# EricPedley/ORB_SLAM3_ROS2

Measured on AMD Instinct MI355X. Metric: frames/sec ORB extract+match @640×480; KF/sec LocalBA (50 KF, 2k pts), higher is better.
Workload: dtype u8; 1 GPU; C2: 640x480, 8-level pyramid, 1000 feat/frame, FAST 20/7, batch=1 per camera stream; ORBextractor::operator() + brute-force Hamming match to the camera's previous frame; step=one frame on each of 16 independent camera streams, parallelism=replicas x1 (no collective); 16 camera streams per GPU, batch 1 each, cameras=16

## Files before the change

orb_slam3_ros2_amd/csrc/extract.cpp:

```cpp
#include "extract.h"

#include <algorithm>
#include <cstdlib>
#include <cstring>
#include <map>
#include <memory>
#include <mutex>
#include <vector>

#include "devbuf.h"
#include "graph_cache.h"
#include "orbhip_kernels.h"
#include "stage.h"

#define HIPOK(x) ORBHIP_HIPOK(" extract", x)

namespace orbhip {
namespace {

struct Plan {
    HostPlan hp;
    DevBuf<ExtractPlan> d_plan;
    DevBuf<CellGeom> d_cells;
    DevBuf<int> d_xofs, d_xalpha, d_yofs, d_ybeta, d_disc, d_cone_tab, d_cone_hi_tab, d_bands, d_flow_dep;
// ... 9 lines not shown
};
std::mutex g_plan_m;
std::map<PlanKey, std::weak_ptr<Plan>>& plan_cache() {
    static auto* m = new std::map<PlanKey, std::weak_ptr<Plan>>();
    return *m;
}

int cone_hi_threads() {
    static const int t = std::getenv("ORBHIP_CONE_HI_THREADS") ? std::atoi(std::getenv("ORBHIP_CONE_HI_THREADS")) : 256;
    return (t == 512 || t == 1024) ? t : 256;
}

template <typename T>
hipError_t upload(DevBuf<T>& d, const std::vector<T>& v) {
    if (v.empty()) return hipSuccess;
    const hipError_t e = d.ensure(v.size());
    return e != hipSuccess ? e : hipMemcpy(d.p, v.data(), v.size() * sizeof(T), hipMemcpyHostToDevice);
}

int upload_plan(Plan& pl) {
    const HostPlan& hp = pl.hp;
    HIPOK(pl.d_plan.ensure(1));
    HIPOK(hipMemcpy(pl.d_plan.p, &hp.h, sizeof(ExtractPlan), hipMemcpyHostToDevice));
    HIPOK(upload(pl.d_cells, hp.cells));
    HIPOK(upload(pl.d_xofs, hp.xofs));
    HIPOK(upload(pl.d_xalpha, hp.xalpha));
    HIPOK(upload(pl.d_yofs, hp.yofs));
    HIPOK(upload(pl.d_ybeta, hp.ybeta));
    HIPOK(upload(pl.d_disc, hp.disc));
    HIPOK(upload(pl.d_otab, hp.otab));
    HIPOK(upload(pl.d_bands, hp.bands));
    HIPOK(upload(pl.d_flow_dep, hp.flow_dep));
    HIPOK(upload(pl.d_cone_hi, hp.cone_hi));
    HIPOK(upload(pl.d_cone_hi_tab, hp.cone_hi_tab));
    HIPOK(upload(pl.d_cone, hp.cone));
    HIPOK(upload(pl.d_cone_tab, hp.cone_tab));
    return ORBHIP_OK;
}

struct RunSwitches {
    int oct_fast, oct_max_dh;
    bool no_cone;
    bool cone_hi;
    bool pack;
    bool flow;
};
RunSwitches read_run_switches() {
    auto is1 = [](const char* name) {
        const char* e = std::getenv(name);
        return e && e[0] == '1';
    };
    const char* e_dh = std::getenv("ORBHIP_OCTREE_DH");
    RunSwitches s;
    s.oct_fast = is1("ORBHIP_OCTREE_SWEEP") ? 0 : 1;
    s.oct_max_dh = e_dh ? std::max(1, std::min(6, std::atoi(e_dh))) : 6;
    s.no_cone = std::getenv("ORBHIP_NO_CONE") != nullptr;
    s.cone_hi = is1("ORBHIP_CONE_HI");
    s.pack = is1("ORBHIP_CAND_PACK");
    s.flow = is1("ORBHIP_RZ_FLOW");
    return s;
}

}

struct ExtractWorkspace {
    int device = 0;
    const orbhip_orb_params* prm = nullptr;
    const OrbTables* tab = nullptr;
    StageTimer* timer = nullptr;
// ... 61 lines not shown
    HIPOK(ws->grow(ws->d_pyr, (size_t)B * P.pyr_bytes));
    HIPOK(ws->grow(ws->d_cand, (size_t)B * P.n_slots_total));
    HIPOK(ws->grow(ws->d_cprim, (size_t)B * P.n_cells_total * kCandPrim));
    HIPOK(ws->grow(ws->d_kscratch, (size_t)B * P.n_slots_total));
    HIPOK(ws->grow(ws->d_nscratch, (size_t)B * P.n_slots_total));
    HIPOK(ws->grow(ws->d_cand_cnt, (size_t)B * P.n_cells_total));
    HIPOK(ws->grow(ws->d_cand_off, (size_t)B * P.n_cells_total));
    HIPOK(ws->grow(ws->d_cand_fill, (size_t)B * kMaxLevels));
    if (pl->hp.flow_nbt) {
        const uint64_t was = ws->gen;
        HIPOK(ws->grow(ws->d_flow, kFlowCtl + (size_t)B * pl->hp.flow_nbt));
        if (ws->gen != was) HIPOK(hipMemset(ws->d_flow.p, 0, ws->d_flow.n * sizeof(int)));
    }
    HIPOK(ws->grow(ws->d_lvl_kp, (size_t)B * P.kp_slots_total));
    HIPOK(ws->grow(ws->d_lvl_cnt, (size_t)B * P.n_levels));
    HIPOK(ws->grow(ws->d_lvl_nlap, (size_t)B * P.n_levels));
    HIPOK(ws->grow(ws->d_err, 4));
    return ORBHIP_OK;
}

static void launch_pyramid(ExtractWorkspace* ws, Plan* pl, FrameBufs& fb, int B, const RunSwitches& sw, bool flow_on,
                           hipStream_t st) {
    const ExtractPlan& P = pl->hp.h;
    StageTimer& tm = *ws->timer;
    static const size_t cone_max = std::getenv("ORBHIP_CONE_MAX_WG")
                                       ? (size_t)std::atol(std::getenv("ORBHIP_CONE_MAX_WG"))
                                       : (size_t)1024;
    const bool cone_path = pl->hp.cone_tiles && !sw.no_cone && (size_t)B * pl->hp.cone_tiles <= cone_max;
    const bool cone_hi = !cone_path && pl->hp.cone_hi_tiles && sw.cone_hi;
    fb.stamp = (cone_path && tm.stage == 1 && tm.dstamp && tm.n < StageTimer::kCap) ? tm.dstamp + tm.n : nullptr;
    if (cone_path) {
        static const int cone_nt = [] {
            const char* e = std::getenv("ORBHIP_CONE_NT");
            const int v = e ? std::atoi(e) : 1024;
            return (v == 256 || v == 512) ? v : 1024;
        }();
        launch_pyr_cone(pl->d_plan.p, pl->hp.cone_tiles, pl->hp.cone_lds, fb, B, pl->d_cone.p, pl->d_cone_tab.p,
                        pl->hp.cone_tab_stride, st, 0, cone_nt, pl->d_xofs.p, pl->d_xalpha.p, pl->d_yofs.p,
                        pl->d_ybeta.p);
    } else if (flow_on) {
        PyrFlow fa{};
        fa.ctl = ws->d_flow.p;
        fa.flags = ws->d_flow.p + kFlowCtl;
        fa.dep = (const int2*)pl->d_flow_dep.p;
        for (int l = 0; l <= kMaxLevels; l++) fa.boff[l] = pl->hp.flow_boff[l];
        fa.B = B;
        fa.nbt = pl->hp.flow_nbt;
        fa.pyr_limit = (int)((int64_t)B * P.pyr_bytes);
        launch_pyr_flow(pl->d_plan.p, fb, pl->d_xofs.p, pl->d_xalpha.p, pl->d_yofs.p, pl->d_ybeta.p, fa, st);
    } else {
        const bool bands = !cone_hi && pl->hp.nbands > 0;
        const int lr = cone_hi ? kConeHiStart + 1 : (bands ? kBandStart + 1 : P.n_levels);
        for (int l = 1; l < lr; l++)
            launch_resize(pl->d_plan.p, P, fb, B, l, pl->d_xofs.p, pl->d_xalpha.p, pl->d_yofs.p, pl->d_ybeta.p,
                          st);
        if (cone_hi)
            launch_pyr_cone(pl->d_plan.p, pl->hp.cone_hi_tiles, pl->hp.cone_hi_lds, fb, B, pl->d_cone_hi.p,
                            pl->d_cone_hi_tab.p, pl->hp.cone_hi_tab_stride, st, kConeHiStart, cone_hi_threads(),
                            pl->d_xofs.p, pl->d_xalpha.p, pl->d_yofs.p, pl->d_ybeta.p);
        if (bands)
            launch_resize_bands(pl->d_plan.p, pl->hp.nbands, fb, B, kBandStart, (const int2*)pl->d_bands.p,
                                pl->d_xofs.p, pl->d_xalpha.p, pl->d_yofs.p, pl->d_ybeta.p, st);
    }
}

static int run_extract(ExtractWorkspace* ws, Plan* pl, const uint8_t* d_imgs, int B, int stride, int64_t fstride,
                       int lap0, int lap1, orbhip_kp* d_kps, uint8_t* d_desc, int cap, int32_t* d_n, int32_t* d_mono,
                       hipStream_t st) {
    const ExtractPlan& P = pl->hp.h;
    (void)hipGetLastError();
    int rc = ensure_batch(ws, pl, B);
    if (rc) return rc;
    const RunSwitches sw = read_run_switches();
    const bool flow_on = sw.flow && pl->hp.flow_nbt > 0 && (int64_t)B * P.pyr_bytes < (1ll << 31);
    GraphKey key;
    key.add(1).add((uint64_t)sw.oct_fast).add((uint64_t)sw.oct_max_dh).add((uint64_t)sw.no_cone)
        .add((uint64_t)sw.cone_hi).add((uint64_t)flow_on).add((uint64_t)sw.pack).add((uint64_t)ws->fast_nt).ptr(pl)
        .ptr(d_imgs).add((uint64_t)B).add((uint64_t)stride).add((uint64_t)fstride).add((uint64_t)lap0)
        .add((uint64_t)lap1).ptr(d_kps).ptr(d_desc).add((uint64_t)cap).ptr(d_n).ptr(d_mono).ptr(st)
        .ptr(ws).add(ws->gen);
    return ws->graphs->run(key, st, ws->timer->stage != 0, [&](hipStream_t st) -> int {
        FrameBufs fb;
        fb.in = d_imgs; fb.in_stride = stride; fb.in_fstride = fstride; fb.pyr = ws->d_pyr.p;
        StageTimer& tm = *ws->timer;
        const StageScope scope(tm);
        tm.begin(1, st);
        launch_pyramid(ws, pl, fb, B, sw, flow_on, st);
        tm.end(1, st);
        tm.begin(2, st);
        CandPack cp;
        cp.prim = ws->d_cprim.p;
// ... 192 lines not shown
```

orb_slam3_ros2_amd/csrc/extract_kernels.hip:

```cpp
#include <hip/hip_runtime.h>
#include <cstdlib>
#include <type_traits>

#include "../../include/orbhip.h"
#include "dev_attr.h"
#include "../../include/orbhip_pattern.h"
#include "orbhip_device.h"
#include "orbhip_kernels.h"
#include "orbhip_plan.h"

namespace orbhip {

__constant__ __attribute__((visibility("hidden"))) signed char kPattern[256 * 4] = ORBHIP_BIT_PATTERN_31_INIT;

ORBHIP_TRACE_UNIT(extract)

struct ImgRef {
    const uint8_t* p;
    int pitch;
};

__device__ __forceinline__ ImgRef level_img(const ExtractPlan* __restrict__ P, const FrameBufs& fb, int f, int l) {
    if (l == 0) return ImgRef{fb.in + (int64_t)f * fb.in_fstride, fb.in_stride};
    return ImgRef{fb.pyr + (int64_t)f * P->pyr_bytes + P->lv[l].pyr_off, P->lv[l].pitch};
// ... 279 lines not shown
                        typedef unsigned int u32x4v __attribute__((ext_vector_type(4)));
                        const u32x4v u = {v.x, v.y, v.z, v.w};
                        __builtin_amdgcn_raw_buffer_store_b128(u, prs, obase + (dyb + r) * pitch + c, 0, 16);
                    }
                    wave_lds_only();
                }
            }
            asm volatile("s_waitcnt vmcnt(0)" ::: "memory");
            __syncthreads();
            if (tid == 0)
                __hip_atomic_store((ex_gint*)(fl + a.boff[l] + b), gen + 1, __ATOMIC_RELAXED,
                                   __HIP_MEMORY_SCOPE_AGENT);
            if (tr_k < 32) { TR_PHASE(7, 2 * tr_k + 1) }
            tr_k++;
        }
    }
    TR_END(7)
    if (tid == 0 && atomicAdd(ctl + kFlowQ, 1) == (int)gridDim.x - 1) {
        for (int i = 0; i <= kFlowQ; i++)
            __hip_atomic_store((ex_gint*)(ctl + i), 0, __ATOMIC_RELAXED, __HIP_MEMORY_SCOPE_AGENT);
        __hip_atomic_store((ex_gint*)(ctl + kFlowQ + 1), gen + 1, __ATOMIC_RELAXED, __HIP_MEMORY_SCOPE_AGENT);
    }
}

__device__ __forceinline__ int small_div(int i, float inv_d) { return (int)(((float)i + 0.5f) * inv_d); }

__device__ __forceinline__ void wait_vm_all() { asm volatile("s_waitcnt vmcnt(0)" ::: "memory"); }
__device__ __forceinline__ void lds_only_barrier() {
    asm volatile("s_waitcnt lgkmcnt(0)" ::: "memory");
    __builtin_amdgcn_s_barrier();
    asm volatile("" ::: "memory");
}

__device__ __forceinline__ void pyr_cone_body(const ExtractPlan* __restrict__ P, const FrameBufs& fb,
                                              const ConeRect* __restrict__ rects, const int* __restrict__ ctab,
                                              int tab_stride, uint8_t* __restrict__ cone, int tile, int f, int s0) {
    TR_BEGIN()
    const int L = P->n_levels, tid = threadIdx.x, nt = blockDim.x;
    const ConeRect* R = rects + (size_t)tile * kMaxLevels;
    static_assert(sizeof(ConeRect) == 16 && kMaxLevels * 4 <= 64 && (kMaxLevels & (kMaxLevels - 1)) == 0, "4 dwords per level");
    const uint32_t rdw = ((const uint32_t*)R)[threadIdx.x & (4 * kMaxLevels - 1)];
    auto rect = [&](int l) -> ConeRect {
        const uint32_t d0 = (uint32_t)__builtin_amdgcn_readlane((int)rdw, 4 * l),
                       d1 = (uint32_t)__builtin_amdgcn_readlane((int)rdw, 4 * l + 1),
                       d2 = (uint32_t)__builtin_amdgcn_readlane((int)rdw, 4 * l + 2),
                       d3 = (uint32_t)__builtin_amdgcn_readlane((int)rdw, 4 * l + 3);
        return ConeRect{(int16_t)(d0 & 0xFFFF), (int16_t)(d0 >> 16), (int16_t)(d1 & 0xFFFF), (int16_t)(d1 >> 16),
                        (int16_t)(d2 & 0xFFFF), (int16_t)(d2 >> 16), (int16_t)(d3 & 0xFFFF), (int16_t)(d3 >> 16)};
    };
    int boff[kMaxLevels], toff[kMaxLevels];
    int tot = 0;
    const ConeRect Rs0 = rect(s0);
    const int P0 = (Rs0.nx1 - Rs0.nx0 + 6) & ~3;
    for (int l = s0; l < L; l++) {
        const ConeRect r = rect(l);
        boff[l] = tot;
        tot += ((l == s0 ? P0 : (r.nx1 - r.nx0)) * (r.ny1 - r.ny0) + 15) & ~15;
    }
    int sh0 = 0;
    int* tab = (int*)(cone + tot);
    int ttot = 0;
    for (int l = s0 + 1; l < L; l++) {
        toff[l] = ttot;
        const ConeRect r = rect(l);
        ttot += 2 * (r.nx1 - r.nx0) + 3 * (r.ny1 - r.ny0);
    }
    const int* gt = ctab + (size_t)tile * tab_stride;
    auto tab_at = [&](int i) -> int { return gt[i]; };
    TR_PHASE(0, 20)
    {
        const ImgRef in0 = level_img(P, fb, f, s0);
        const ConeRect r = Rs0;
        const int nw = r.nx1 - r.nx0, nh = r.ny1 - r.ny0;
        const uint8_t* src0 = in0.p + (int64_t)r.ny0 * in0.pitch + r.nx0;
        const bool dw = ((in0.pitch & 3) == 0) && ((((uintptr_t)in0.p) & 3) == 0);
        if (dw) sh0 = (int)(((uintptr_t)src0) & 3);
        const int nwd = dw ? (nw + sh0 + 3) >> 2 : 0;
        const int tot0 = dw ? nwd * nh : nw * nh;
        const float inv_n = 1.0f / (float)(dw ? nwd : nw);
        uint8_t* lv0 = cone + boff[s0];
        if (dw && tot0 <= 1024 && ttot <= 2 * 1024 && nt == 1024) {
            const uint32_t* s4 = (const uint32_t*)(src0 - sh0);
            const int p4 = in0.pitch >> 2;
            int tv[2];
#pragma unroll
            for (int u = 0; u < 2; u++) tv[u] = gt[min(tid + 1024 * u, ttot - 1)];
            const int i = min(tid, tot0 - 1);
            const int y = small_div(i, inv_n), x = i - y * nwd;
            const uint32_t v = s4[(int64_t)y * p4 + x];
#pragma unroll
            for (int u = 0; u < 2; u++)
                if (tid + 1024 * u < ttot) tab[tid + 1024 * u] = tv[u];
            if (tid < tot0) ((uint32_t*)lv0)[y * (P0 >> 2) + x] = v;
            TR_PHASE(0, 21)
        } else if (dw) {
            const uint32_t* s4 = (const uint32_t*)(src0 - sh0);
            const int p4 = in0.pitch >> 2;
            constexpr int U = 8;
            for (int i0 = tid; i0 < ttot; i0 += U * nt) {
                int v[U];
#pragma unroll
                for (int u = 0; u < U; u++) v[u] = tab_at(min(i0 + u * nt, ttot - 1));
#pragma unroll
                for (int u = 0; u < U; u++)
                    if (i0 + u * nt < ttot) tab[i0 + u * nt] = v[u];
            }
            for (int i0 = tid; i0 < tot0; i0 += U * nt) {
                uint32_t v[U];
                int o[U];
#pragma unroll
                for (int u = 0; u < U; u++) {
                    const int i = min(i0 + u * nt, tot0 - 1);
                    const int y = small_div(i, inv_n), x = i - y * nwd;
                    v[u] = s4[(int64_t)y * p4 + x];
                    o[u] = y * (P0 >> 2) + x;
                }
#pragma unroll
                for (int u = 0; u < U; u++)
                    if (i0 + u * nt < tot0) ((uint32_t*)lv0)[o[u]] = v[u];
            }
        } else {
            for (int i = tid; i < ttot; i += nt) tab[i] = tab_at(i);
            for (int i = tid; i < tot0; i += nt) {
                const int y = small_div(i, inv_n), x = i - y * nw;
                lv0[y * P0 + x] = src0[(int64_t)y * in0.pitch + x];
            }
        }
    }
    __syncthreads();
    TR_PHASE(0, 0)
    for (int l = s0 + 1; l < L; l++) {
        const LevelGeom& D = P->lv[l];
        const ConeRect r = rect(l), rp = rect(l - 1);
        const int nw = r.nx1 - r.nx0, nh = r.ny1 - r.ny0, nwp = l == s0 + 1 ? P0 : rp.nx1 - rp.nx0;
        const int* t = tab + toff[l];
        const uint8_t* src = cone + boff[l - 1] + (l == s0 + 1 ? sh0 : 0);
        uint8_t* dst = fb.pyr + (int64_t)f * P->pyr_bytes + D.pyr_off;
        const float inv_nw = 1.0f / (float)nw;
        const bool noclamp = D.rz_noclamp != 0;
        for (int i = tid; i < nw * nh; i += nt) {
            const int yy = small_div(i, inv_nw), xx = i - yy * nw;
            const int x = r.nx0 + xx, y = r.ny0 + yy;
            const int sx = t[xx] - rp.nx0;
            const uint8_t* S0 = src + (t[2 * nw + 3 * yy] - rp.ny0) * nwp;
            const uint8_t* S1 = src + (t[2 * nw + 3 * yy + 1] - rp.ny0) * nwp;
            int h0, h1;
            if (x < D.xmax) {
                const int aa = t[nw + xx];
                const int a0 = (int)(short)(aa & 0xFFFF), a1 = (int)(short)(aa >> 16);
                h0 = S0[sx] * a0 + S0[sx + 1] * a1;
                h1 = S1[sx] * a0 + S1[sx + 1] * a1;
            } else {
                h0 = S0[sx] * 2048;
                h1 = S1[sx] * 2048;
            }
            const int bb = t[2 * nw + 3 * yy + 2];
            const int b0 = (int)(short)(bb & 0xFFFF), b1 = (int)(short)(bb >> 16);
            int v;
            if (x < D.vend && noclamp) {
                v = ((__mul24(h0 >> 4, b0) >> 16) + (__mul24(h1 >> 4, b1) >> 16) + 2) >> 2;
            } else if (x < D.vend) {
                int s0 = min(max(h0 >> 4, -32768), 32767);
                int s1 = min(max(h1 >> 4, -32768), 32767);
                int tt = ((s0 * b0) >> 16) + ((s1 * b1) >> 16);
                tt = min(max(tt, -32768), 32767);
                v = (tt + 2) >> 2;
            } else {
                v = (h0 * b0 + h1 * b1 + (1 << 21)) >> 22;
            }
            const uint8_t u = (uint8_t)(v < 0 ? 0 : (v > 255 ? 255 : v));
            cone[boff[l] + i] = u;
            if (x >= r.ox0 && x < r.ox1 && y >= r.oy0 && y < r.oy1) dst[(int64_t)y * D.pitch + x] = u;
        }
        lds_only_barrier();
        TR_PHASE(0, l)
    }
    TR_END(0)
}

__global__ __launch_bounds__(1024) void k_pyr_cone(const ExtractPlan* __restrict__ P, FrameBufs fb,
                                                   const ConeRect* __restrict__ rects, const int* __restrict__ ctab,
                                                   int tab_stride, int xrun, int s0) {
    extern __shared__ __attribute__((aligned(16))) uint8_t cone[];
    if (fb.stamp && threadIdx.x == 0) atomicMin(fb.stamp, (unsigned long long)__builtin_amdgcn_s_memrealtime());
    const int X = gridDim.x, lg = xcd_runs(blockIdx.x + X * blockIdx.y, X * gridDim.y, xrun < 0 ? X : xrun);
    pyr_cone_body(P, fb, rects, ctab, tab_stride, cone, lg % X, lg / X, s0);
    if (fb.stamp) {
        __syncthreads();
        if (threadIdx.x == 0) atomicMax(fb.stamp + kStampStride, (unsigned long long)__builtin_amdgcn_s_memrealtime());
    }
}

constexpr int kWinMax = 80;
#ifndef ORBHIP_OCT_W0_MAIN
#define ORBHIP_OCT_W0_MAIN 1
#endif
#ifndef ORBHIP_OCT_BLK_FINAL
#define ORBHIP_OCT_BLK_FINAL 1
#endif
typedef _Float16 h2 __attribute__((ext_vector_type(2)));
typedef unsigned short u16x2 __attribute__((ext_vector_type(2)));
constexpr uint32_t kPwBias = 0x64006400u;

__device__ __forceinline__ h2 as_h2(uint32_t u) { return __builtin_bit_cast(h2, u); }
__device__ __forceinline__ h2 hmin(h2 a, h2 b) { return __builtin_elementwise_minimum(a, b); }
__device__ __forceinline__ h2 hmax(h2 a, h2 b) { return __builtin_elementwise_maximum(a, b); }

template <int P>
// ... 1174 lines not shown
                const int rank = lap ? before : p - before;
                LevelKp r;
                r.x = (int16_t)x; r.y = (int16_t)y;
                r.srl = (uint32_t)sc | ((uint32_t)lap << 8) | ((uint32_t)rank << 9);
                out[p] = r;
            }
            lap_run += tot;
        }
        if (tid == 0) {
            lvl_cnt[f * P->n_levels + l] = ncap;
            lvl_nlap[f * P->n_levels + l] = lap_run;
            if (n > G.kp_cap) atomicOr(err, 2);
        }
        return true;
    };
    if (Dh) {
        if (run(std::true_type{})) {
            TR_PHASE(2, 63)
            TR_END(2)
            stamp_end();
            return;
        }
        for (int i = tid; i < nIni * 4; i += nt) S.ccount[i] = 0;
        __syncthreads();
    }
    run(std::false_type{});
    TR_PHASE(2, 63)
    TR_END(2)
    stamp_end();
}

constexpr int kBlR = 18, kBlW = 2 * kBlR + 1;
constexpr int kDpP = 48;
constexpr int kHrP = 48;
__device__ __forceinline__ constexpr uint32_t blur_tap(int i) {
    return i == 0 || i == 6 ? 18u : (i == 1 || i == 5 ? 34u : (i == 2 || i == 4 ? 48u : 56u));
}
__device__ __forceinline__ bool desc_dword_span_ok(int cx, int cy, int lw, int lh) {
    return ((cx - kPatchR) & ~3) + kDpP <= ((lw + 3) & ~3) || cy + kPatchR + 1 < lh;
}

__global__ __launch_bounds__(256) void k_desc(const ExtractPlan* __restrict__ P, FrameBufs fb,
                                              const LevelKp* __restrict__ lvl_kp, const int* __restrict__ lvl_cnt,
                                              const int* __restrict__ lvl_nlap, const int* __restrict__ disc,
                                              orbhip_kp* __restrict__ out_kps, uint8_t* __restrict__ out_desc,
                                              int cap, int* __restrict__ n_out, int* __restrict__ mono_out, int xrun) {
    __shared__ __attribute__((aligned(16))) uint8_t patch[4][kPatchW * kDpP + 16];
    __shared__ __attribute__((aligned(16))) uint16_t hrow[4][kBlW * kHrP];
    TR_BEGIN()
    const int X = gridDim.x, lg = xcd_runs(blockIdx.x + X * blockIdx.y, X * gridDim.y, xrun < 0 ? X : xrun);
    const int f = lg / X;
    const int wid = threadIdx.x >> 6, lane = threadIdx.x & 63;
    int slot = (lg % X) * 4 + wid;
    const int L = P->n_levels;
    int total = 0, nlap_tot = 0;
    for (int l = 0; l < L; l++) { total += lvl_cnt[f * L + l]; nlap_tot += lvl_nlap[f * L + l]; }
    if (lg % X == 0 && threadIdx.x == 0) {
        n_out[f] = total;
        mono_out[f] = total - nlap_tot;
    }
    int l = 0, mono_base = 0, lap_base = 0;
    while (l < L && slot >= P->lv[l].kp_cap) {
        slot -= P->lv[l].kp_cap;
        mono_base += lvl_cnt[f * L + l] - lvl_nlap[f * L + l];
        lap_base += lvl_nlap[f * L + l];
        l++;
    }
// ... 475 lines not shown
```

orb_slam3_ros2_amd/csrc/extract_plan.cpp:

```cpp
#include "extract_plan.h"

#include <algorithm>
#include <cfloat>
#include <cstdio>
#include <cstdlib>

namespace orbhip {

static int round_even_d(double v) { return (int)std::nearbyint(v); }
static int floor_f(float v) { int i = (int)v; return i - (i > v); }
static short sat_s16(int v) { return (short)std::min(std::max(v, -32768), 32767); }

OrbTables build_orb_tables(const orbhip_orb_params& prm) {
    OrbTables t;
    const int L = prm.n_levels;
    const double sf = (double)prm.scale_factor;
    t.scale.assign(L, 1.f);
    t.inv_scale.assign(L, 1.f);
    for (int i = 1; i < L; i++) t.scale[i] = (float)(t.scale[i - 1] * sf);
    for (int i = 0; i < L; i++) t.inv_scale[i] = 1.0f / t.scale[i];
    t.feat.assign(L, 0);
    const float factor = (float)(1.0f / sf);
    float nd = prm.n_features * (1 - factor) / (1 - (float)std::pow((double)factor, (double)L));
    int sum = 0;
// ... 17 lines not shown
    const int n = 7, n2 = 3;
    double vals[3], s = 0, scale2X = -0.125 / (2.0 * 2.0);
    for (int i = 0, x = 1 - n; i < n2; i++, x += 2) { vals[i] = std::exp((double)(x * x) * scale2X); s += vals[i]; }
    s = s * 2 + 1.0;
    const double mul1 = 1.0 / s;
    double err = 0;
    long tot = 0;
    for (int i = 0; i < n2; i++) {
        double adj = vals[i] * mul1 * 256.0 + err;
        long v0 = round_even_d(adj);
        err = adj - (double)v0;
        t.blurk[i] = t.blurk[n - 1 - i] = (int)v0;
        tot += v0;
    }
    t.blurk[n2] = (int)(256 - 2 * tot);
    return t;
}

PlanSwitches read_plan_switches(int cone_tile_hint) {
    auto env = [](const char* name, int unset, int lo) {
        const char* e = std::getenv(name);
        return e ? std::max(lo, std::atoi(e)) : unset;
    };
    PlanSwitches s{};
    const int ts = env("ORBHIP_CONE_TILE", 0, 0);
    s.cone_tile = ts > 0 ? ts : (cone_tile_hint > 0 ? cone_tile_hint : 10);
    s.cone_hi_tile = env("ORBHIP_CONE_HI_TILE", 32, 4);
    s.rz_bands = env("ORBHIP_RZ_BANDS", 0, 0);
    s.clist_cap = env("ORBHIP_FAST_CLIST_CAP", -1, 0);
    s.fast_nt = env("ORBHIP_FAST_NT", -1, 0);
    return s;
}

static int cone_tables(const ExtractPlan& P, const HostPlan& pl, int s0, int ts, std::vector<ConeRect>& rects,
                       std::vector<int>& ctab, size_t& tab_stride, size_t& lds_max) {
    const int L = P.n_levels;
    const LevelGeom& T = P.lv[L - 1];
    const int ntx = (T.w + ts - 1) / ts, nty = (T.h + ts - 1) / ts;
    lds_max = 0;
    rects.assign((size_t)ntx * nty * kMaxLevels, ConeRect{});
    auto source_of = [&](int l, int nx0, int nx1, int ny0, int ny1, int* a0, int* a1, int* b0, int* b1) {
        const LevelGeom& U = P.lv[l];
        const LevelGeom& G = P.lv[l - 1];
        *a0 = pl.xofs[U.xtab_off + nx0];
        *a1 = pl.xofs[U.xtab_off + nx1 - 1] + ((nx1 - 1) < U.xmax ? 1 : 0) + 1;
        auto clampr = [&](int r) { return r < 0 ? 0 : (r < G.h ? r : G.h - 1); };
        *b0 = clampr(pl.yofs[U.ytab_off + ny0]);
        *b1 = clampr(pl.yofs[U.ytab_off + ny1 - 1] + 1) + 1;
    };
    for (int ti = 0; ti < nty; ti++)
        for (int tj = 0; tj < ntx; tj++) {
            ConeRect* R = &rects[((size_t)ti * ntx + tj) * kMaxLevels];
            int nx0 = 0, nx1 = 0, ny0 = 0, ny1 = 0;
            for (int l = L - 1; l > s0; l--) {
                const LevelGeom& G = P.lv[l];
                const int ox0 = (int)((int64_t)tj * G.w / ntx), ox1 = (int)((int64_t)(tj + 1) * G.w / ntx);
                const int oy0 = (int)((int64_t)ti * G.h / nty), oy1 = (int)((int64_t)(ti + 1) * G.h / nty);
                int a0 = ox0, a1 = ox1, b0 = oy0, b1 = oy1;
                if (l < L - 1 && nx1 > nx0 && ny1 > ny0) {
                    int lo, hi, r0, r1;
                    source_of(l + 1, nx0, nx1, ny0, ny1, &lo, &hi, &r0, &r1);
                    a0 = std::min(a0, lo); a1 = std::max(a1, hi);
                    b0 = std::min(b0, r0); b1 = std::max(b1, r1);
                    if (ox1 <= ox0 || oy1 <= oy0) { a0 = lo; a1 = hi; b0 = r0; b1 = r1; }
                }
                R[l] = ConeRect{(int16_t)a0, (int16_t)a1, (int16_t)b0, (int16_t)b1,
                                (int16_t)ox0, (int16_t)ox1, (int16_t)oy0, (int16_t)oy1};
                nx0 = a0; nx1 = a1; ny0 = b0; ny1 = b1;
            }
            {
                int lo, hi, r0, r1;
                source_of(s0 + 1, nx0, nx1, ny0, ny1, &lo, &hi, &r0, &r1);
                R[s0] = ConeRect{(int16_t)lo, (int16_t)hi, (int16_t)r0, (int16_t)r1, 0, 0, 0, 0};
            }
            size_t tot = 0, ttot = 0;
            for (int l = s0; l < L; l++) {
                const size_t wl = l == s0 ? (size_t)((R[s0].nx1 - R[s0].nx0 + 6) & ~3) : (size_t)(R[l].nx1 - R[l].nx0);
                tot += (wl * (R[l].ny1 - R[l].ny0) + 15) & ~size_t(15);
            }
            for (int l = s0 + 1; l < L; l++)
                ttot += 4 * (2 * (size_t)(R[l].nx1 - R[l].nx0) + 3 * (size_t)(R[l].ny1 - R[l].ny0));
            lds_max = std::max(lds_max, tot + ttot);
        }
    tab_stride = 0;
    for (int t = 0; t < ntx * nty; t++) {
        size_t tt = 0;
        for (int l = s0 + 1; l < L; l++) {
            const ConeRect& r = rects[(size_t)t * kMaxLevels + l];
            tt += 2 * (size_t)(r.nx1 - r.nx0) + 3 * (size_t)(r.ny1 - r.ny0);
        }
        tab_stride = std::max(tab_stride, tt);
    }
    ctab.assign((size_t)ntx * nty * tab_stride, 0);
    for (int t = 0; t < ntx * nty; t++) {
        int* o = ctab.data() + (size_t)t * tab_stride;
        for (int l = s0 + 1; l < L; l++) {
            const LevelGeom& D = P.lv[l];
            const LevelGeom& S = P.lv[l - 1];
            const ConeRect r = rects[(size_t)t * kMaxLevels + l];
            const int nw = r.nx1 - r.nx0, nh = r.ny1 - r.ny0;
            for (int i = 0; i < nw; i++) {
                o[i] = pl.xofs[D.xtab_off + r.nx0 + i];
                o[nw + i] = pl.xalpha[D.xtab_off + r.nx0 + i];
            }
            auto clampr = [&](int v) { return v < 0 ? 0 : (v < S.h ? v : S.h - 1); };
            for (int j = 0; j < nh; j++) {
                const int sy = pl.yofs[D.ytab_off + r.ny0 + j];
                o[2 * nw + 3 * j] = clampr(sy);
                o[2 * nw + 3 * j + 1] = clampr(sy + 1);
                o[2 * nw + 3 * j + 2] = pl.ybeta[D.ytab_off + r.ny0 + j];
            }
            o += 2 * nw + 3 * nh;
        }
    }
    return ntx * nty;
}
int plan_build_host(const orbhip_orb_params& prm, const OrbTables& tab, int w, int h, const PlanSwitches& sw,
                    HostPlan& out) {
    out = HostPlan();
    ExtractPlan& P = out.h;
    const int L = prm.n_levels;
    P.w = w; P.h = h; P.n_levels = L;
    P.ini_th = std::min(std::max(prm.ini_th_fast, 0), 255);
    P.min_th = std::min(std::max(prm.min_th_fast, 0), 255);
    P.clist_cap = sw.clist_cap < 0 ? kClistCap : std::min(sw.clist_cap, kClistCap);
    P.fast_nt = 0;
    if (sw.fast_nt >= 0) {
        const int v = sw.fast_nt;
        if (v == 128 || v == 256 || v == 512 || v == 1024) P.fast_nt = v;
        else std::fprintf(stderr, "orbhip: ORBHIP_FAST_NT=%d ignored (128, 256, 512 or 1024)\n", v);
    }
    for (int i = 0; i < 7; i++) P.blurk[i] = tab.blurk[i];
    static const int kTaps[7] = {18, 34, 48, 56, 48, 34, 18};
    for (int i = 0; i < 7; i++)
        if (P.blurk[i] != kTaps[i]) return ORBHIP_ERR_UNSUPPORTED;
    int64_t pyr_off = 0;
    int cell_base = 0, slot_base = 0, kp_base = 0, max_cells = 0, hc_max = 7, wc_max = 7;
    for (int l = 0; l < L; l++) {
        LevelGeom& G = P.lv[l];
        G.w = round_even_f((float)w * tab.inv_scale[l]);
        G.h = round_even_f((float)h * tab.inv_scale[l]);
        if (G.w < 64 || G.h < 64) return ORBHIP_ERR_UNSUPPORTED;
        G.pitch = l == 0 ? 0 : ((G.w + 63) / 64) * 64;
        G.pyr_off = l == 0 ? 0 : pyr_off;
        if (l > 0) pyr_off += (int64_t)G.pitch * G.h;
// ... 98 lines not shown
        kp_base += G.kp_cap;
        if ((G.max_bx - G.min_bx) >= 4096 || (G.max_by - G.min_by) >= 4096) return ORBHIP_ERR_UNSUPPORTED;
        {
            auto bits6 = [](int v, int a0, int a1) {
                int b = 0;
                for (int d = 0; d < 6; d++) {
                    const int sv = a0 + (int)std::ceil((float)(a1 - a0) / 2);
                    const bool hi = v >= sv;
                    (hi ? a0 : a1) = sv;
                    b = 2 * b + (hi ? 1 : 0);
                }
                return b;
            };
            const int Wl = G.max_bx - G.min_bx, Hl = G.max_by - G.min_by;
            G.oct_tab_off = (int)out.otab.size();
            for (int x = 0; x < Wl; x++) {
                int r = (int)((float)x / G.hX);
                r = r < 0 ? 0 : (r >= G.n_ini ? G.n_ini - 1 : r);
                out.otab.push_back((uint16_t)((r << 8) | bits6(x, (int)(G.hX * (float)r), (int)(G.hX * (float)(r + 1)))));
            }
            for (int y = 0; y < Hl; y++) out.otab.push_back((uint16_t)bits6(y, 0, Hl));
        }
    }
    P.n_cells_total = cell_base;
    P.n_slots_total = slot_base;
    P.kp_slots_total = kp_base;
    P.pyr_bytes = ((pyr_off + 255) / 256) * 256;
    P.max_cells_level = max_cells;
    out.kp_cap_frame = kp_base;
    P.fast_win_rows = hc_max;
    P.fast_win_cols = wc_max;
    if (L > 1) {
        std::vector<ConeRect> rects;
        std::vector<int> ctab;
        size_t stride = 0, lds = 0;
        const int ts = sw.cone_tile;
        int tiles = cone_tables(P, out, 0, ts, rects, ctab, stride, lds);
        if (lds <= 60 * 1024) {
            out.cone_tab.swap(ctab);
            out.cone_tab_stride = (int)stride;
            out.cone.swap(rects);
            out.cone_tiles = tiles;
            out.cone_lds = lds;
        }
        if (L > kConeHiStart + 1) {
            tiles = cone_tables(P, out, kConeHiStart, sw.cone_hi_tile, rects, ctab, stride, lds);
            if (lds <= 60 * 1024) {
                out.cone_hi_tab.swap(ctab);
                out.cone_hi_tab_stride = (int)stride;
                out.cone_hi.swap(rects);
                out.cone_hi_tiles = tiles;
                out.cone_hi_lds = lds;
            }
        }
    }
    {
        const int nb = std::min(sw.rz_bands, L > 0 ? P.lv[L - 1].h : 0);
        if (L > kBandStart + 1 && nb > 0) {
            out.bands.assign((size_t)nb * kMaxLevels * 2, 0);
            for (int b = 0; b < nb; b++) {
                int n0 = 0, n1 = 0;
                for (int l = L - 1; l > kBandStart; l--) {
                    const LevelGeom& G = P.lv[l];
                    int r0 = (int)((int64_t)b * G.h / nb), r1 = (int)((int64_t)(b + 1) * G.h / nb);
                    if (l < L - 1 && n1 > n0) {
                        const LevelGeom& U = P.lv[l + 1];
                        auto clampr = [&](int r) { return r < 0 ? 0 : (r < G.h ? r : G.h - 1); };
                        const int s0r = clampr(out.yofs[U.ytab_off + n0]);
                        const int s1r = clampr(out.yofs[U.ytab_off + n1 - 1] + 1) + 1;
                        if (r1 > r0) { r0 = std::min(r0, s0r); r1 = std::max(r1, s1r); }
                        else { r0 = s0r; r1 = s1r; }
                    }
                    out.bands[((size_t)b * kMaxLevels + l) * 2] = r0;
                    out.bands[((size_t)b * kMaxLevels + l) * 2 + 1] = r1;
                    n0 = r0; n1 = r1;
                }
            }
            out.nbands = nb;
        }
    }
    if (L > 1) {
        constexpr int kFR = 16, kGroup = 4, kSrcRows = 6;
// ... 54 lines not shown
```

orb_slam3_ros2_amd/csrc/extract_plan.h:

```cpp
#pragma once
#include <cmath>
#include <vector>

#include "../../include/orbhip.h"
#include "orbhip_plan.h"

namespace orbhip {

constexpr int kConeHiStart = 2;
constexpr int kBandStart = 2;

inline int round_even_f(float v) { return (int)std::nearbyintf(v); }

struct OrbTables {
    std::vector<float> scale, inv_scale;
    std::vector<int> feat, umax;
    int blurk[7] = {0};
};
OrbTables build_orb_tables(const orbhip_orb_params& prm);

struct PlanSwitches {
    int cone_tile;
    int cone_hi_tile;
    int rz_bands;
    int clist_cap;
    int fast_nt;
};
PlanSwitches read_plan_switches(int cone_tile_hint);

struct HostPlan {
    ExtractPlan h{};
    std::vector<CellGeom> cells;
    std::vector<int> xofs, xalpha, yofs, ybeta, disc;
    std::vector<uint16_t> otab;
    std::vector<ConeRect> cone;
    std::vector<int> cone_tab;
    int cone_tab_stride = 0, cone_tiles = 0;
    size_t cone_lds = 0;
    std::vector<ConeRect> cone_hi;
    std::vector<int> cone_hi_tab;
    int cone_hi_tab_stride = 0, cone_hi_tiles = 0;
    size_t cone_hi_lds = 0;
    std::vector<int> bands;
    int nbands = 0;
    int flow_boff[kMaxLevels + 1] = {0};
    int flow_nbt = 0;
    std::vector<int> flow_dep;
    OctreeCfg oct{};
    int kp_cap_frame = 0;
};

int plan_build_host(const orbhip_orb_params& prm, const OrbTables& tab, int w, int h, const PlanSwitches& sw,
                    HostPlan& out);

}
```

Before: 43870 frames/s.

## Vectorize pyramid cone kernel to four pixels per thread with padded run tables

Rebuilds the per-tile cone resize tables host-side into a padded, int4-aligned layout: rows are rounded to multiples of four and the row entries are padded to four ints. The cone kernel now has each thread produce four output pixels. It gathers source bytes with dword loads, v_perm and sdot2, stores packed dwords, and loads the tables as int4. Per-level geometry is broadcast through readlane instead of scalar loads. The default cone thread count drops from 1024 to 512, and the descriptor blur scratch pitch changes from 48 to 46 halfwords to spread LDS banks. This adds LDS padding, alignment constraints and more complex boundary handling.

```diff
diff --git a/orb_slam3_ros2_amd/csrc/extract.cpp b/orb_slam3_ros2_amd/csrc/extract.cpp
--- a/orb_slam3_ros2_amd/csrc/extract.cpp
+++ b/orb_slam3_ros2_amd/csrc/extract.cpp
@@ -65,9 +65,9 @@
     HIPOK(upload(pl.d_bands, hp.bands));
     HIPOK(upload(pl.d_flow_dep, hp.flow_dep));
     HIPOK(upload(pl.d_cone_hi, hp.cone_hi));
-    HIPOK(upload(pl.d_cone_hi_tab, hp.cone_hi_tab));
+    HIPOK(upload(pl.d_cone_hi_tab, hp.cone_hi_run_tab));
     HIPOK(upload(pl.d_cone, hp.cone));
-    HIPOK(upload(pl.d_cone_tab, hp.cone_tab));
+    HIPOK(upload(pl.d_cone_tab, hp.cone_run_tab));
     return ORBHIP_OK;
 }
 
@@ -195,11 +195,11 @@
     if (cone_path) {
         static const int cone_nt = [] {
             const char* e = std::getenv("ORBHIP_CONE_NT");
-            const int v = e ? std::atoi(e) : 1024;
-            return (v == 256 || v == 512) ? v : 1024;
+            const int v = e ? std::atoi(e) : 512;
+            return (v == 256 || v == 1024) ? v : 512;
         }();
         launch_pyr_cone(pl->d_plan.p, pl->hp.cone_tiles, pl->hp.cone_lds, fb, B, pl->d_cone.p, pl->d_cone_tab.p,
-                        pl->hp.cone_tab_stride, st, 0, cone_nt, pl->d_xofs.p, pl->d_xalpha.p, pl->d_yofs.p,
+                        pl->hp.cone_run_stride, st, 0, cone_nt, pl->d_xofs.p, pl->d_xalpha.p, pl->d_yofs.p,
                         pl->d_ybeta.p);
     } else if (flow_on) {
         PyrFlow fa{};
@@ -219,7 +219,7 @@
                           st);
         if (cone_hi)
             launch_pyr_cone(pl->d_plan.p, pl->hp.cone_hi_tiles, pl->hp.cone_hi_lds, fb, B, pl->d_cone_hi.p,
-                            pl->d_cone_hi_tab.p, pl->hp.cone_hi_tab_stride, st, kConeHiStart, cone_hi_threads(),
+                            pl->d_cone_hi_tab.p, pl->hp.cone_hi_run_stride, st, kConeHiStart, cone_hi_threads(),
                             pl->d_xofs.p, pl->d_xalpha.p, pl->d_yofs.p, pl->d_ybeta.p);
         if (bands)
             launch_resize_bands(pl->d_plan.p, pl->hp.nbands, fb, B, kBandStart, (const int2*)pl->d_bands.p,
diff --git a/orb_slam3_ros2_amd/csrc/extract_kernels.hip b/orb_slam3_ros2_amd/csrc/extract_kernels.hip
--- a/orb_slam3_ros2_amd/csrc/extract_kernels.hip
+++ b/orb_slam3_ros2_amd/csrc/extract_kernels.hip
@@ -335,6 +335,8 @@
     asm volatile("" ::: "memory");
 }
 
+typedef short s16x2 __attribute__((ext_vector_type(2)));
+
 __device__ __forceinline__ void pyr_cone_body(const ExtractPlan* __restrict__ P, const FrameBufs& fb,
                                               const ConeRect* __restrict__ rects, const int* __restrict__ ctab,
                                               int tab_stride, uint8_t* __restrict__ cone, int tile, int f, int s0) {
@@ -351,25 +353,28 @@
         return ConeRect{(int16_t)(d0 & 0xFFFF), (int16_t)(d0 >> 16), (int16_t)(d1 & 0xFFFF), (int16_t)(d1 >> 16),
                         (int16_t)(d2 & 0xFFFF), (int16_t)(d2 >> 16), (int16_t)(d3 & 0xFFFF), (int16_t)(d3 >> 16)};
     };
-    int boff[kMaxLevels], toff[kMaxLevels];
-    int tot = 0;
+    static_assert(kMaxLevels * 4 == 64, "one lane per (level, field)");
+    const LevelGeom& Gl = P->lv[(threadIdx.x & 63) >> 2];
+    const int gfld = threadIdx.x & 3;
+    const uint32_t gdw = gfld == 0 ? (uint32_t)Gl.pyr_off
+                                   : (gfld == 1 ? (uint32_t)Gl.pitch
+                                                : (gfld == 2 ? ((uint32_t)Gl.xmax | (uint32_t)Gl.vend << 16)
+                                                             : (uint32_t)Gl.rz_noclamp));
+    uint8_t* const pyr_f = fb.pyr + (int64_t)f * P->pyr_bytes;
     const ConeRect Rs0 = rect(s0);
     const int P0 = (Rs0.nx1 - Rs0.nx0 + 6) & ~3;
-    for (int l = s0; l < L; l++) {
+    const int bytes0 = (P0 * (Rs0.ny1 - Rs0.ny0) + 15) & ~15;
+    int tot = bytes0, ttot = 0;
+    for (int l = s0 + 1; l < L; l++) {
         const ConeRect r = rect(l);
-        boff[l] = tot;
-        tot += ((l == s0 ? P0 : (r.nx1 - r.nx0)) * (r.ny1 - r.ny0) + 15) & ~15;
+        const int nwp = (r.nx1 - r.nx0 + 3) & ~3, nh = r.ny1 - r.ny0;
+        tot += (nwp * nh + 15) & ~15;
+        ttot += 2 * nwp + 4 * nh;
     }
     int sh0 = 0;
     int* tab = (int*)(cone + tot);
-    int ttot = 0;
-    for (int l = s0 + 1; l < L; l++) {
-        toff[l] = ttot;
-        const ConeRect r = rect(l);
-        ttot += 2 * (r.nx1 - r.nx0) + 3 * (r.ny1 - r.ny0);
-    }
-    const int* gt = ctab + (size_t)tile * tab_stride;
-    auto tab_at = [&](int i) -> int { return gt[i]; };
+    const int4* gt = (const int4*)(ctab + (size_t)tile * tab_stride);
+    const int tq = ttot >> 2;
     TR_PHASE(0, 20)
     {
         const ImgRef in0 = level_img(P, fb, f, s0);
@@ -381,32 +386,38 @@
         const int nwd = dw ? (nw + sh0 + 3) >> 2 : 0;
         const int tot0 = dw ? nwd * nh : nw * nh;
         const float inv_n = 1.0f / (float)(dw ? nwd : nw);
-        uint8_t* lv0 = cone + boff[s0];
-        if (dw && tot0 <= 1024 && ttot <= 2 * 1024 && nt == 1024) {
+        uint8_t* lv0 = cone;
+        constexpr int US = 4;
+        if (dw && tot0 <= US * nt && tq <= nt) {
             const uint32_t* s4 = (const uint32_t*)(src0 - sh0);
             const int p4 = in0.pitch >> 2;
-            int tv[2];
-#pragma unroll
-            for (int u = 0; u < 2; u++) tv[u] = gt[min(tid + 1024 * u, ttot - 1)];
-            const int i = min(tid, tot0 - 1);
-            const int y = small_div(i, inv_n), x = i - y * nwd;
-            const uint32_t v = s4[(int64_t)y * p4 + x];
-#pragma unroll
-            for (int u = 0; u < 2; u++)
-                if (tid + 1024 * u < ttot) tab[tid + 1024 * u] = tv[u];
-            if (tid < tot0) ((uint32_t*)lv0)[y * (P0 >> 2) + x] = v;
+            const int4 tv = gt[min(tid, tq - 1)];
+            uint32_t v[US];
+            int o[US];
+#pragma unroll
+            for (int u = 0; u < US; u++)
+                if (u * nt < tot0) {
+                    const int i = min(tid + u * nt, tot0 - 1);
+                    const int y = small_div(i, inv_n), x = i - y * nwd;
+                    v[u] = s4[(int64_t)y * p4 + x];
+                    o[u] = y * (P0 >> 2) + x;
+                }
+            if (tid < tq) ((int4*)tab)[tid] = tv;
+#pragma unroll
+            for (int u = 0; u < US; u++)
+                if (tid + u * nt < tot0) ((uint32_t*)lv0)[o[u]] = v[u];
             TR_PHASE(0, 21)
         } else if (dw) {
             const uint32_t* s4 = (const uint32_t*)(src0 - sh0);
             const int p4 = in0.pitch >> 2;
             constexpr int U = 8;
-            for (int i0 = tid; i0 < ttot; i0 += U * nt) {
-                int v[U];
-#pragma unroll
-                for (int u = 0; u < U; u++) v[u] = tab_at(min(i0 + u * nt, ttot - 1));
+            for (int i0 = tid; i0 < tq; i0 += U * nt) {
+                int4 v[U];
+#pragma unroll
+                for (int u = 0; u < U; u++) v[u] = gt[min(i0 + u * nt, tq - 1)];
 #pragma unroll
                 for (int u = 0; u < U; u++)
-                    if (i0 + u * nt < ttot) tab[i0 + u * nt] = v[u];
+                    if (i0 + u * nt < tq) ((int4*)tab)[i0 + u * nt] = v[u];
             }
             for (int i0 = tid; i0 < tot0; i0 += U * nt) {
                 uint32_t v[U];
@@ -423,7 +434,7 @@
                     if (i0 + u * nt < tot0) ((uint32_t*)lv0)[o[u]] = v[u];
             }
         } else {
-            for (int i = tid; i < ttot; i += nt) tab[i] = tab_at(i);
+            for (int i = tid; i < tq; i += nt) ((int4*)tab)[i] = gt[i];
             for (int i = tid; i < tot0; i += nt) {
                 const int y = small_div(i, inv_n), x = i - y * nw;
                 lv0[y * P0 + x] = src0[(int64_t)y * in0.pitch + x];
@@ -432,51 +443,87 @@
     }
     __syncthreads();
     TR_PHASE(0, 0)
+    int bsrc = 0, bdst = bytes0, to = 0;
+    int srcp = P0, nx0p = Rs0.nx0 - sh0, ny0p = Rs0.ny0;
     for (int l = s0 + 1; l < L; l++) {
-        const LevelGeom& D = P->lv[l];
-        const ConeRect r = rect(l), rp = rect(l - 1);
-        const int nw = r.nx1 - r.nx0, nh = r.ny1 - r.ny0, nwp = l == s0 + 1 ? P0 : rp.nx1 - rp.nx0;
-        const int* t = tab + toff[l];
-        const uint8_t* src = cone + boff[l - 1] + (l == s0 + 1 ? sh0 : 0);
-        uint8_t* dst = fb.pyr + (int64_t)f * P->pyr_bytes + D.pyr_off;
-        const float inv_nw = 1.0f / (float)nw;
-        const bool noclamp = D.rz_noclamp != 0;
-        for (int i = tid; i < nw * nh; i += nt) {
-            const int yy = small_div(i, inv_nw), xx = i - yy * nw;
-            const int x = r.nx0 + xx, y = r.ny0 + yy;
-            const int sx = t[xx] - rp.nx0;
-            const uint8_t* S0 = src + (t[2 * nw + 3 * yy] - rp.ny0) * nwp;
-            const uint8_t* S1 = src + (t[2 * nw + 3 * yy + 1] - rp.ny0) * nwp;
-            int h0, h1;
-            if (x < D.xmax) {
-                const int aa = t[nw + xx];
-                const int a0 = (int)(short)(aa & 0xFFFF), a1 = (int)(short)(aa >> 16);
-                h0 = S0[sx] * a0 + S0[sx + 1] * a1;
-                h1 = S1[sx] * a0 + S1[sx + 1] * a1;
+        const ConeRect r = rect(l);
+        const int nw = r.nx1 - r.nx0, nh = r.ny1 - r.ny0, nq = (nw + 3) >> 2, nwp = 4 * nq;
+        const int* t = tab + to;
+        const uint8_t* src = cone + bsrc;
+        uint32_t* out = (uint32_t*)(cone + bdst);
+        const uint32_t g2 = (uint32_t)__builtin_amdgcn_readlane((int)gdw, 4 * l + 2);
+        const int pitch = __builtin_amdgcn_readlane((int)gdw, 4 * l + 1);
+        const int xmax = (int)(g2 & 0xFFFF), vend = (int)(g2 >> 16);
+        const bool noclamp = __builtin_amdgcn_readlane((int)gdw, 4 * l + 3) != 0;
+        uint8_t* dst = pyr_f + (uint32_t)__builtin_amdgcn_readlane((int)gdw, 4 * l);
+        const float inv_nq = 1.0f / (float)nq;
+        for (int i = tid; i < nq * nh; i += nt) {
+            const int yy = small_div(i, inv_nq), q = i - yy * nq;
+            const int4 re = *(const int4*)(t + 2 * nwp + 4 * yy);
+            const int4 xo4 = *(const int4*)(t + 4 * q), xa4 = *(const int4*)(t + nwp + 4 * q);
+            const int xo[4] = {xo4.x, xo4.y, xo4.z, xo4.w}, xa[4] = {xa4.x, xa4.y, xa4.z, xa4.w};
+            const int x0 = r.nx0 + 4 * q, y = r.ny0 + yy;
+            const uint8_t* S0 = src + (re.x - ny0p) * srcp;
+            const uint8_t* S1 = src + (re.y - ny0p) * srcp;
+            const int b0 = (int)(short)(re.z & 0xFFFF), b1 = (int)(short)(re.z >> 16);
+            int h0[4], h1[4], v[4];
+            uint32_t w0[4][2], w1[4][2], sel[4];
+#pragma unroll
+            for (int k = 0; k < 4; k++) {
+                const int c = xo[k] - nx0p;
+                sel[k] = 0x0c010c00u + 0x00010001u * (uint32_t)(c & 3);
+                const uint32_t* p0 = (const uint32_t*)(S0 + (c & ~3));
+                const uint32_t* p1 = (const uint32_t*)(S1 + (c & ~3));
+                w0[k][0] = p0[0]; w0[k][1] = p0[1];
+                w1[k][0] = p1[0]; w1[k][1] = p1[1];
+            }
+#pragma unroll
+            for (int k = 0; k < 4; k++) {
+                const int aa = x0 + k < xmax ? xa[k] : 2048;
+                const s16x2 a2 = __builtin_bit_cast(s16x2, aa);
+                h0[k] = __builtin_amdgcn_sdot2(__builtin_bit_cast(s16x2, __builtin_amdgcn_perm(w0[k][1], w0[k][0], sel[k])), a2, 0, false);
+                h1[k] = __builtin_amdgcn_sdot2(__builtin_bit_cast(s16x2, __builtin_amdgcn_perm(w1[k][1], w1[k][0], sel[k])), a2, 0, false);
+            }
+            if (noclamp) {
+#pragma unroll
+                for (int k = 0; k < 4; k++)
+                    v[k] = ((__mul24(h0[k] >> 4, b0) >> 16) + (__mul24(h1[k] >> 4, b1) >> 16) + 2) >> 2;
             } else {
-                h0 = S0[sx] * 2048;
-                h1 = S1[sx] * 2048;
-            }
-            const int bb = t[2 * nw + 3 * yy + 2];
-            const int b0 = (int)(short)(bb & 0xFFFF), b1 = (int)(short)(bb >> 16);
-            int v;
-            if (x < D.vend && noclamp) {
-                v = ((__mul24(h0 >> 4, b0) >> 16) + (__mul24(h1 >> 4, b1) >> 16) + 2) >> 2;
-            } else if (x < D.vend) {
-                int s0 = min(max(h0 >> 4, -32768), 32767);
-                int s1 = min(max(h1 >> 4, -32768), 32767);
-                int tt = ((s0 * b0) >> 16) + ((s1 * b1) >> 16);
-                tt = min(max(tt, -32768), 32767);
-                v = (tt + 2) >> 2;
-            } else {
-                v = (h0 * b0 + h1 * b1 + (1 << 21)) >> 22;
-            }
-            const uint8_t u = (uint8_t)(v < 0 ? 0 : (v > 255 ? 255 : v));
-            cone[boff[l] + i] = u;
-            if (x >= r.ox0 && x < r.ox1 && y >= r.oy0 && y < r.oy1) dst[(int64_t)y * D.pitch + x] = u;
+#pragma unroll
+                for (int k = 0; k < 4; k++) {
+                    const int s0 = min(max(h0[k] >> 4, -32768), 32767);
+                    const int s1 = min(max(h1[k] >> 4, -32768), 32767);
+                    int tt = ((s0 * b0) >> 16) + ((s1 * b1) >> 16);
+                    tt = min(max(tt, -32768), 32767);
+                    v[k] = (tt + 2) >> 2;
+                }
+            }
+            if (x0 + 3 >= vend) {
+#pragma unroll
+                for (int k = 0; k < 4; k++)
+                    if (x0 + k >= vend) v[k] = (h0[k] * b0 + h1[k] * b1 + (1 << 21)) >> 22;
+            }
+            uint32_t pk = 0;
+#pragma unroll
+            for (int k = 0; k < 4; k++) pk |= (uint32_t)min(max(v[k], 0), 255) << (8 * k);
+            out[i] = pk;
+            if (y >= r.oy0 && y < r.oy1) {
+                uint8_t* d = dst + y * pitch + x0;
+                if (x0 >= r.ox0 && x0 + 4 <= r.ox1) {
+                    *(uint32_t*)d = pk;
+                } else {
+#pragma unroll
+                    for (int k = 0; k < 4; k++)
+                        if (x0 + k >= r.ox0 && x0 + k < r.ox1) d[k] = (uint8_t)(pk >> (8 * k));
+                }
+            }
         }
         lds_only_barrier();
         TR_PHASE(0, l)
+        bsrc = bdst;
+        bdst += (nwp * nh + 15) & ~15;
+        to += 2 * nwp + 4 * nh;
+        srcp = nwp; nx0p = r.nx0; ny0p = r.ny0;
     }
     TR_END(0)
 }
@@ -1717,7 +1764,12 @@
 
 constexpr int kBlR = 18, kBlW = 2 * kBlR + 1;
 constexpr int kDpP = 48;
-constexpr int kHrP = 48;
+constexpr int kHrP = 46;
+static_assert(kHrP % 2 == 0, "the column pass reads row pairs as aligned dwords");
+static_assert(kHrP >= 46, "the column pass reads halfwords r0 .. r0 + 9, r0 <= 36");
+static_assert((kHrP / 2) % 2 == 1, "an odd dword pitch spreads the columns over the LDS banks");
+static_assert((kBlW * kHrP * sizeof(uint16_t)) % 4 == 0 && kBlW * kHrP * sizeof(uint16_t) <= 4 * 1024,
+              "k_desc holds one buffer per wave, each dword aligned");
 __device__ __forceinline__ constexpr uint32_t blur_tap(int i) {
     return i == 0 || i == 6 ? 18u : (i == 1 || i == 5 ? 34u : (i == 2 || i == 4 ? 48u : 56u));
 }
diff --git a/orb_slam3_ros2_amd/csrc/extract_plan.cpp b/orb_slam3_ros2_amd/csrc/extract_plan.cpp
--- a/orb_slam3_ros2_amd/csrc/extract_plan.cpp
+++ b/orb_slam3_ros2_amd/csrc/extract_plan.cpp
@@ -73,12 +73,18 @@
     return s;
 }
 
+static size_t round4(size_t v) { return (v + 3) & ~size_t(3); }
+static size_t cone_run_ints(int nw, int nh) { return 2 * round4((size_t)nw) + 4 * (size_t)nh; }
 static int cone_tables(const ExtractPlan& P, const HostPlan& pl, int s0, int ts, std::vector<ConeRect>& rects,
-                       std::vector<int>& ctab, size_t& tab_stride, size_t& lds_max) {
+                       std::vector<int>& ctab, size_t& tab_stride, std::vector<int>& rtab, size_t& rtab_stride,
+                       size_t& lds_max) {
     const int L = P.n_levels;
     const LevelGeom& T = P.lv[L - 1];
     const int ntx = (T.w + ts - 1) / ts, nty = (T.h + ts - 1) / ts;
     lds_max = 0;
+    rects.clear(); ctab.clear(); rtab.clear();
+    tab_stride = rtab_stride = 0;
+    if (P.pyr_bytes >= (int64_t(1) << 31)) return 0;
     rects.assign((size_t)ntx * nty * kMaxLevels, ConeRect{});
     auto source_of = [&](int l, int nx0, int nx1, int ny0, int ny1, int* a0, int* a1, int* b0, int* b1) {
         const LevelGeom& U = P.lv[l];
@@ -105,6 +111,7 @@
                     b0 = std::min(b0, r0); b1 = std::max(b1, r1);
                     if (ox1 <= ox0 || oy1 <= oy0) { a0 = lo; a1 = hi; b0 = r0; b1 = r1; }
                 }
+                a0 &= ~3;
                 R[l] = ConeRect{(int16_t)a0, (int16_t)a1, (int16_t)b0, (int16_t)b1,
                                 (int16_t)ox0, (int16_t)ox1, (int16_t)oy0, (int16_t)oy1};
                 nx0 = a0; nx1 = a1; ny0 = b0; ny1 = b1;
@@ -114,27 +121,24 @@
                 source_of(s0 + 1, nx0, nx1, ny0, ny1, &lo, &hi, &r0, &r1);
                 R[s0] = ConeRect{(int16_t)lo, (int16_t)hi, (int16_t)r0, (int16_t)r1, 0, 0, 0, 0};
             }
-            size_t tot = 0, ttot = 0;
+            size_t tot = 0, ttot = 0, rtot = 0;
             for (int l = s0; l < L; l++) {
-                const size_t wl = l == s0 ? (size_t)((R[s0].nx1 - R[s0].nx0 + 6) & ~3) : (size_t)(R[l].nx1 - R[l].nx0);
+                const size_t wl = l == s0 ? (size_t)((R[s0].nx1 - R[s0].nx0 + 6) & ~3) : round4(R[l].nx1 - R[l].nx0);
                 tot += (wl * (R[l].ny1 - R[l].ny0) + 15) & ~size_t(15);
             }
-            for (int l = s0 + 1; l < L; l++)
-                ttot += 4 * (2 * (size_t)(R[l].nx1 - R[l].nx0) + 3 * (size_t)(R[l].ny1 - R[l].ny0));
-            lds_max = std::max(lds_max, tot + ttot);
-        }
-    tab_stride = 0;
-    for (int t = 0; t < ntx * nty; t++) {
-        size_t tt = 0;
-        for (int l = s0 + 1; l < L; l++) {
-            const ConeRect& r = rects[(size_t)t * kMaxLevels + l];
-            tt += 2 * (size_t)(r.nx1 - r.nx0) + 3 * (size_t)(r.ny1 - r.ny0);
-        }
-        tab_stride = std::max(tab_stride, tt);
-    }
+            for (int l = s0 + 1; l < L; l++) {
+                ttot += 2 * (size_t)(R[l].nx1 - R[l].nx0) + 3 * (size_t)(R[l].ny1 - R[l].ny0);
+                rtot += cone_run_ints(R[l].nx1 - R[l].nx0, R[l].ny1 - R[l].ny0);
+            }
+            lds_max = std::max(lds_max, tot + 4 * rtot);
+            tab_stride = std::max(tab_stride, ttot);
+            rtab_stride = std::max(rtab_stride, rtot);
+        }
     ctab.assign((size_t)ntx * nty * tab_stride, 0);
+    rtab.assign((size_t)ntx * nty * rtab_stride, 0);
     for (int t = 0; t < ntx * nty; t++) {
         int* o = ctab.data() + (size_t)t * tab_stride;
+        int* q = rtab.data() + (size_t)t * rtab_stride;
         for (int l = s0 + 1; l < L; l++) {
             const LevelGeom& D = P.lv[l];
             const LevelGeom& S = P.lv[l - 1];
@@ -151,7 +155,17 @@
                 o[2 * nw + 3 * j + 1] = clampr(sy + 1);
                 o[2 * nw + 3 * j + 2] = pl.ybeta[D.ytab_off + r.ny0 + j];
             }
+            const int nwp = (int)round4(nw);
+            for (int i = 0; i < nwp; i++) {
+                q[i] = o[std::min(i, nw - 1)];
+                q[nwp + i] = o[nw + std::min(i, nw - 1)];
+            }
+            for (int j = 0; j < nh; j++) {
+                for (int k = 0; k < 3; k++) q[2 * nwp + 4 * j + k] = o[2 * nw + 3 * j + k];
+                q[2 * nwp + 4 * j + 3] = 0;
+            }
             o += 2 * nw + 3 * nh;
+            q += cone_run_ints(nw, nh);
         }
     }
     return ntx * nty;
@@ -316,22 +330,26 @@
     P.fast_win_cols = wc_max;
     if (L > 1) {
         std::vector<ConeRect> rects;
-        std::vector<int> ctab;
-        size_t stride = 0, lds = 0;
+        std::vector<int> ctab, rtab;
+        size_t stride = 0, rstride = 0, lds = 0;
         const int ts = sw.cone_tile;
-        int tiles = cone_tables(P, out, 0, ts, rects, ctab, stride, lds);
-        if (lds <= 60 * 1024) {
+        int tiles = cone_tables(P, out, 0, ts, rects, ctab, stride, rtab, rstride, lds);
+        if (tiles && lds <= 60 * 1024) {
             out.cone_tab.swap(ctab);
             out.cone_tab_stride = (int)stride;
+            out.cone_run_tab.swap(rtab);
+            out.cone_run_stride = (int)rstride;
             out.cone.swap(rects);
             out.cone_tiles = tiles;
             out.cone_lds = lds;
         }
         if (L > kConeHiStart + 1) {
-            tiles = cone_tables(P, out, kConeHiStart, sw.cone_hi_tile, rects, ctab, stride, lds);
-            if (lds <= 60 * 1024) {
+            tiles = cone_tables(P, out, kConeHiStart, sw.cone_hi_tile, rects, ctab, stride, rtab, rstride, lds);
+            if (tiles && lds <= 60 * 1024) {
                 out.cone_hi_tab.swap(ctab);
                 out.cone_hi_tab_stride = (int)stride;
+                out.cone_hi_run_tab.swap(rtab);
+                out.cone_hi_run_stride = (int)rstride;
                 out.cone_hi.swap(rects);
                 out.cone_hi_tiles = tiles;
                 out.cone_hi_lds = lds;
diff --git a/orb_slam3_ros2_amd/csrc/extract_plan.h b/orb_slam3_ros2_amd/csrc/extract_plan.h
--- a/orb_slam3_ros2_amd/csrc/extract_plan.h
+++ b/orb_slam3_ros2_amd/csrc/extract_plan.h
@@ -34,12 +34,12 @@
     std::vector<int> xofs, xalpha, yofs, ybeta, disc;
     std::vector<uint16_t> otab;
     std::vector<ConeRect> cone;
-    std::vector<int> cone_tab;
-    int cone_tab_stride = 0, cone_tiles = 0;
+    std::vector<int> cone_tab, cone_run_tab;
+    int cone_tab_stride = 0, cone_run_stride = 0, cone_tiles = 0;
     size_t cone_lds = 0;
     std::vector<ConeRect> cone_hi;
-    std::vector<int> cone_hi_tab;
-    int cone_hi_tab_stride = 0, cone_hi_tiles = 0;
+    std::vector<int> cone_hi_tab, cone_hi_run_tab;
+    int cone_hi_tab_stride = 0, cone_hi_run_stride = 0, cone_hi_tiles = 0;
     size_t cone_hi_lds = 0;
     std::vector<int> bands;
     int nbands = 0;
```

New measurement: 48550 frames/s, median of 4. 1.11x the previous value.
